# ZhongLingXiao/nano-kazen

Hardware: AMD Instinct MI355X
Metric: Msamples/s (w*h*spp/s) at 1920x1080, 1 M-tri scene (higher is better)
Workload: dtype f32

## Files before the change

nano-kazen_amd/csrc/kz_devfn.h:

```cpp
#pragma once
#include <hip/hip_runtime.h>
#include "kz_internal.h"
#include "kz_crmath.h"

#define KZ_BLOCK 256
#define KZ_INF __builtin_huge_valf()

struct V3 { float x, y, z; };
__device__ __forceinline__ V3 mk(float x, float y, float z) { V3 r; r.x = x; r.y = y; r.z = z; return r; }
__device__ __forceinline__ V3 mk(float a) { return mk(a, a, a); }
__device__ __forceinline__ V3 operator+(V3 a, V3 b) { return mk(a.x + b.x, a.y + b.y, a.z + b.z); }
__device__ __forceinline__ V3 operator-(V3 a, V3 b) { return mk(a.x - b.x, a.y - b.y, a.z - b.z); }
__device__ __forceinline__ V3 operator-(V3 a) { return mk(-a.x, -a.y, -a.z); }
__device__ __forceinline__ V3 operator*(V3 a, float s) { return mk(a.x * s, a.y * s, a.z * s); }
__device__ __forceinline__ V3 operator*(float s, V3 a) { return mk(a.x * s, a.y * s, a.z * s); }
__device__ __forceinline__ V3 operator*(V3 a, V3 b) { return mk(a.x * b.x, a.y * b.y, a.z * b.z); }
__device__ __forceinline__ V3 operator/(V3 a, float s) { return mk(a.x / s, a.y / s, a.z / s); }
__device__ __forceinline__ float dot(V3 a, V3 b) { return a.x * b.x + a.y * b.y + a.z * b.z; }
__device__ __forceinline__ V3 cross(V3 a, V3 b) { return mk(a.y * b.z - a.z * b.y, a.z * b.x - a.x * b.z, a.x * b.y - a.y * b.x); }
__device__ __forceinline__ float norm(V3 a) { return sqrtf(dot(a, a)); }
__device__ __forceinline__ V3 normalized(V3 a) { float n2 = dot(a, a); return n2 > 0.f ? a / sqrtf(n2) : a; }
__device__ __forceinline__ float maxCoeff(V3 a) { return fmaxf(a.x, fmaxf(a.y, a.z)); }
__device__ __forceinline__ float sqr(float x) { return x * x; }

// ... 64 lines not shown
    do {
        i ^= p; i *= 0xe170893d; i ^= p >> 16; i ^= (i & w) >> 4; i ^= p >> 8;
        i *= 0x0929eb3f; i ^= p >> 23; i ^= (i & w) >> 1; i *= 1 | p >> 27;
        i *= 0x6935fa69; i ^= (i & w) >> 11; i *= 0x74dcb303; i ^= (i & w) >> 2;
        i *= 0x9e501cc3; i ^= (i & w) >> 2; i *= 0xc860a3df; i &= w; i ^= i >> 5;
    } while (i >= l);
    if ((l & w) == 0) return (i + p) & w;
    return (i + p) % l;
}

struct Sampler {
    uint64_t state, inc;
    int px, py; uint32_t idx, dim;
    int type;
    uint64_t hp;

    __device__ __forceinline__ uint32_t nextUInt() {
        uint64_t old = state;
        state = old * PCG32_MULT + inc;
        uint32_t xs = (uint32_t)(((old >> 18u) ^ old) >> 27u);
        uint32_t rot = (uint32_t)(old >> 59u);
        return (xs >> rot) | (xs << ((~rot + 1u) & 31));
    }
    __device__ __forceinline__ float nextFloat() { return __uint_as_float((nextUInt() >> 9) | 0x3f800000u) - 1.0f; }
    __device__ __forceinline__ void generateSample(const KzParams &P, const KzDevTables &T, int x, int y, uint32_t sampleIndex) {
        px = x; py = y; idx = sampleIndex;
        hp = type != KZ_SAMPLER_INDEPENDENT ? hashPixelBlock(x, y) : 0ull;
        if (type != KZ_SAMPLER_PMJ02BN) {
            dim = 0;
            uint64_t h = hashPixelSeed(x, y, P.seed);
// ... 3 lines not shown
            state = state * PCG32_MULT + inc;
            KzPcgJump j = T.jump[sampleIndex];
            state = j.mult * state + inc * j.plus;
        } else {
            dim = 2;
        }
    }
    __device__ __forceinline__ float blueNoise(const KzDevTables &T, uint32_t tex) const {
        uint32_t t = tex % KZ_BLUENOISE_TEXTURES;
        uint32_t x = (uint32_t)px % KZ_BLUENOISE_RES, y = (uint32_t)py % KZ_BLUENOISE_RES;
        return T.bn[(t * KZ_BLUENOISE_RES + x) * KZ_BLUENOISE_RES + y];
    }
    __device__ __forceinline__ float next1D(const KzParams &P, const KzDevTables &T) {
        if (type == KZ_SAMPLER_INDEPENDENT) return nextFloat();
        if (type == KZ_SAMPLER_STRATIFIED) {
            const uint64_t h = hashDimSeed(hp, dim, P.seed);
            const int stratum = (int)permuteIdx(idx, P.sampleCount, (uint32_t)h);
            ++dim;
            const float delta = nextFloat();
            return ((float)stratum + delta) / (float)P.sampleCount;
        }
        if (type == KZ_SAMPLER_CORRELATED) {
            const uint64_t h = hashDimSeed(hp, dim, P.seed);
            const int p = (int)permuteIdx(idx, P.sampleCount, (uint32_t)h * 0x45fbe943u);
            const float j = nextFloat();
            ++dim;
            return ((float)p + j) / (float)P.sampleCount;
        }
        uint64_t h = hashDimSeed(hp, dim, P.seed);
        int index = (int)permuteIdx(idx, P.sampleCount, (uint32_t)h);
        float delta = blueNoise(T, dim);
        ++dim;
        const float num = (float)index + delta;
        return fminf(P.sppPow2 ? num * P.invSpp : num / (float)P.sampleCount, KZ_ONE_MINUS_EPS);
    }
    __device__ __forceinline__ void next2D(const KzParams &P, const KzDevTables &T, float &x, float &y) {
        if (type == KZ_SAMPLER_INDEPENDENT) { y = nextFloat(); x = nextFloat(); return; }
        if (type == KZ_SAMPLER_STRATIFIED) {
            const uint64_t h = hashDimSeed(hp, dim, P.seed);
            const int stratum = (int)permuteIdx(idx, P.sampleCount, (uint32_t)h);
            dim += 2;
            const int sx = stratum % P.resX, sy = stratum / P.resX;
            const float dx = nextFloat();
            const float dy = nextFloat();
            x = ((float)sx + dx) / (float)P.resX; y = ((float)sy + dy) / (float)P.resX;
            return;
        }
        if (type == KZ_SAMPLER_CORRELATED) {
            const uint32_t h = (uint32_t)hashDimSeed(hp, dim, P.seed);
            const uint32_t s = permuteIdx(idx, P.sampleCount, h * 0x51633e2du);
            const uint32_t cy = s / (uint32_t)P.resX, cx = s % (uint32_t)P.resX;
            const uint32_t sx = permuteIdx(cx, (uint32_t)P.resX, h * 0x68bc21ebu);
            const uint32_t sy = permuteIdx(cy, (uint32_t)P.resY, h * 0x02e5be93u);
            const float jx = nextFloat();
            const float jy = nextFloat();
            dim += 2;
            x = ((float)cx + ((float)sy + jx) / (float)P.resY) / (float)P.resX;
            y = ((float)cy + ((float)sx + jy) / (float)P.resX) / (float)P.resY;
            return;
        }
        uint32_t index = idx;
        uint32_t inst = dim / 2;
        if (inst >= KZ_PMJ02BN_SETS) {
            uint64_t h = hashDimSeed(hp, dim, P.seed);
            index = permuteIdx(idx, P.sampleCount, (uint32_t)h);
        }
        inst %= KZ_PMJ02BN_SETS; index %= KZ_PMJ02BN_SAMPLES;
        const float2 e = reinterpret_cast<const float2 *>(T.pmj)[(size_t)inst * KZ_PMJ02BN_SAMPLES + index];
        float ux = e.x, uy = e.y;
        ux += blueNoise(T, dim); uy += blueNoise(T, dim + 1);
        if (ux >= 1) ux -= 1;
        if (uy >= 1) uy -= 1;
        dim += 2;
        x = fminf(ux, KZ_ONE_MINUS_EPS); y = fminf(uy, KZ_ONE_MINUS_EPS);
    }
    __device__ __forceinline__ void nextPixel2D(const KzParams &P, const KzDevTables &T, float &x, float &y) {
        if (type != KZ_SAMPLER_PMJ02BN) { next2D(P, T, x, y); return; }
        int tile = P.pixelTileSize;
        int tx = px % tile, ty = py % tile;
// ... 43 lines not shown
    const float4 *tp = reinterpret_cast<const float4 *>(tri);
    return triTestV(tp[0], tp[1], tp[2], o, d, tmin, tmax, t, u, v, gid);
}
typedef float kz_f4v __attribute__((ext_vector_type(4)));
__device__ __forceinline__ float4 kzLoadStream(const float4 *p) { const kz_f4v v = __builtin_nontemporal_load(reinterpret_cast<const kz_f4v *>(p)); return make_float4(v.x, v.y, v.z, v.w); }
__device__ __forceinline__ void kzStoreStream(float4 *p, float4 v) { const kz_f4v t = {v.x, v.y, v.z, v.w}; __builtin_nontemporal_store(t, reinterpret_cast<kz_f4v *>(p)); }
__device__ __forceinline__ uint32_t kzLoadStream(const uint32_t *p) { return __builtin_nontemporal_load(p); }

typedef __attribute__((address_space(3))) uint32_t KzLds32;
__device__ __forceinline__ uint32_t kzLdsAddr(const uint32_t *p) { return (uint32_t)(uintptr_t)(const KzLds32 *)p; }
__device__ __forceinline__ void kzLdsPut(uint32_t a, uint32_t v) { *(KzLds32 *)(uintptr_t)a = v; }
__device__ __forceinline__ uint32_t kzLdsGet(uint32_t a) { return *(const KzLds32 *)(uintptr_t)a; }

struct Node4Test { uint32_t k0, k1, k2, k3; uint4 refs; };
typedef float kz_f2 __attribute__((ext_vector_type(2)));
__device__ __forceinline__ void node4KeysOf(const uint4 q0, const uint4 q1, const uint4 q2, V3 o, float rx, float ry, float rz, float tmin, float tmax,
                                            uint32_t (&key)[4]) {
    const float ax = __uint_as_float(q0.w) * rx, ay = __uint_as_float(q2.z) * ry, az = __uint_as_float(q2.w) * rz;
    const float bx = (__uint_as_float(q0.x) - o.x) * rx, by = (__uint_as_float(q0.y) - o.y) * ry, bz = (__uint_as_float(q0.z) - o.z) * rz;
    const uint32_t nX = rx >= 0.f ? q1.x : q1.w, fX = rx >= 0.f ? q1.w : q1.x;
    const uint32_t nY = ry >= 0.f ? q1.y : q2.x, fY = ry >= 0.f ? q2.x : q1.y;
    const uint32_t nZ = rz >= 0.f ? q1.z : q2.y, fZ = rz >= 0.f ? q2.y : q1.z;
    const kz_f2 AX = {ax, ax}, AY = {ay, ay}, AZ = {az, az}, BX = {bx, bx}, BY = {by, by}, BZ = {bz, bz};
#pragma unroll
    for (int i = 0; i < 4; ++i) {
        const kz_f2 qx = {(float)((nX >> (8 * i)) & 0xffu), (float)((fX >> (8 * i)) & 0xffu)};
        const kz_f2 qy = {(float)((nY >> (8 * i)) & 0xffu), (float)((fY >> (8 * i)) & 0xffu)};
        const kz_f2 qz = {(float)((nZ >> (8 * i)) & 0xffu), (float)((fZ >> (8 * i)) & 0xffu)};
        const kz_f2 tx = __builtin_elementwise_fma(qx, AX, BX), ty = __builtin_elementwise_fma(qy, AY, BY), tz = __builtin_elementwise_fma(qz, AZ, BZ);
        const float n = fmaxf(fmaxf(fmaxf(tx.x, ty.x), tz.x), tmin);
        const float f = fminf(fminf(fminf(tx.y, ty.y), tz.y) * 1.0000004f, tmax);
        key[i] = (n <= f) ? ((__float_as_uint(n) & ~3u) | (uint32_t)i) : 0xFFFFFFFFu;
    }
}
__device__ __forceinline__ const uint4 *kzNode4Ptr(const KzDevTables &T, uint32_t node) {
    return reinterpret_cast<const uint4 *>(reinterpret_cast<const char *>(T.nodes4) + (uint32_t)(node << 6));
}
__device__ __forceinline__ void node4Keys(const KzDevTables &T, uint32_t node, V3 o, float rx, float ry, float rz, float tmin, float tmax,
                                          uint32_t (&key)[4], uint4 &refs) {
    const uint4 *np = kzNode4Ptr(T, node);
    const uint4 q0 = np[0], q1 = np[1], q2 = np[2];
    refs = np[3];
    node4KeysOf(q0, q1, q2, o, rx, ry, rz, tmin, tmax, key);
}
__device__ __forceinline__ Node4Test node4Test(const KzDevTables &T, uint32_t node, V3 o, float rx, float ry, float rz, float tmin, float tmax) {
    Node4Test r; uint32_t key[4];
    node4Keys(T, node, o, rx, ry, rz, tmin, tmax, key, r.refs);
    uint32_t a = min(key[0], key[1]), b = max(key[0], key[1]), c = min(key[2], key[3]), d = max(key[2], key[3]);
    uint32_t lo = min(a, c), m1 = max(a, c), m2 = min(b, d), hi = max(b, d);
    r.k0 = lo; r.k1 = min(m1, m2); r.k2 = max(m1, m2); r.k3 = hi;
    return r;
}
__device__ __forceinline__ uint32_t pick4b(const uint4 &v, uint32_t i) {
    const bool b0 = i & 1u, b1 = i & 2u;
    const uint32_t lo = b0 ? v.y : v.x, hi = b0 ? v.w : v.z;
    return b1 ? hi : lo;
}
__device__ __forceinline__ uint32_t pick4(const uint4 &v, uint32_t i) { return i == 0 ? v.x : (i == 1 ? v.y : (i == 2 ? v.z : v.w)); }

__device__ __forceinline__ bool rayIsFinite(V3 o, V3 d) { return fabsf(o.x) + fabsf(o.y) + fabsf(o.z) + fabsf(d.x) + fabsf(d.y) + fabsf(d.z) < KZ_INF; }

template <bool STATS>
__device__ __forceinline__ bool closestHit(const KzDevTables &T, uint32_t rootRef, V3 o, V3 d, float tmin, float tmax,
                                           RawHit &best, uint32_t *stk, Counters &cn) {
    bool found = false;
    best.t = KZ_INF; best.u = best.v = 0.f; best.tri = 0; best.gid = 0;
    if (STATS) cn.rays++;
    if (rootRef == 0xFFFFFFFFu) return false;
    if (!(fabsf(o.x) + fabsf(o.y) + fabsf(o.z) + fabsf(d.x) + fabsf(d.y) + fabsf(d.z) < KZ_INF)) return false;
    const float rx = rcpExact(d.x), ry = rcpExact(d.y), rz = rcpExact(d.z);
    uint32_t cur = rootRef;
// ... 971 lines not shown
```

nano-kazen_amd/csrc/kz_render.hip:

```cpp
#include <hip/hip_runtime.h>

#include "kz_internal.h"
#include "kz_devfn.h"
#include "kz_wavefront.h"
#include "kz_integrators.h"
#include "kz_plan.h"
#include <algorithm>
#include <atomic>
#include <chrono>
#include <cmath>
#include <cstdio>
#include <cstdlib>
#include <cstring>
#include <mutex>
#include <string>
#include <thread>
#include <vector>

template <bool STATS, int EXT>
__global__ __launch_bounds__(KZ_BLOCK) void kz_path_megakernel(KzParams P, KzDevTables T, const uint32_t *__restrict__ pixList,
                                                               uint32_t nItems, uint32_t S, uint32_t sampleBegin, const uint32_t *__restrict__ itemSample,
                                                               float *__restrict__ outJx, float *__restrict__ outJy, float *__restrict__ outR,
                                                               float *__restrict__ outG, float *__restrict__ outB,
                                                               unsigned long long *__restrict__ stats) {
// ... 560 lines not shown
                HIP_TRY(hipStreamSynchronize(stream));
                if (left == 0) break;
            }
            trace(0, nextQ, nextCount, 0u, nextCount + 2, nullptr, nullptr);
            { int rc_ = stageMark(c, stream, 1); if (rc_) return rc_; }
            cur = nextQ; curCount = nextCount;
        }
    } else {
        const bool beside = P.nLights > 0 && maxDepth > 1 && (shadowBeside == 2 || (shadowBeside == 0 && items <= KZ_BESIDE_ITEMS));
        ds->lastInfo.shadowBeside = beside ? 1u : 0u;
        if (beside && !c.side) {
            HIP_TRY(hipStreamCreateWithFlags(&c.side, hipStreamNonBlocking));
            HIP_TRY(hipEventCreateWithFlags(&c.evFork, hipEventDisableTiming));
            HIP_TRY(hipEventCreateWithFlags(&c.evJoin, hipEventDisableTiming));
        }
        for (int iter = 0; iter < maxDepth; ++iter) {
            uint32_t *nextQ = W.queue[iter & 1], *nextCount = W.counts + 4 * (iter + 1), *shQ = W.queue[2], *shCount = W.counts + 4 * (iter + 1) + 1;
#define KZ_SHADE(ST, EX) hipLaunchKernelGGL((kz_wf_shade<ST, EX>), gShade, blk, 0, stream, P, Tsh, W, pixList, Sp, sBegin, iter, cur, curCount, items, nextQ, nextCount, shQ, shCount)
            const int xsel = P.bsdfExt == 0 ? 0 : (P.bsdfExt == KZ_X_MODELS ? KZ_X_MODELS : KZ_X_ALL);
            if (st) { if (xsel == KZ_X_ALL) KZ_SHADE(true, KZ_X_ALL); else if (xsel) KZ_SHADE(true, KZ_X_MODELS); else KZ_SHADE(true, 0); }
            else { if (xsel == KZ_X_ALL) KZ_SHADE(false, KZ_X_ALL); else if (xsel) KZ_SHADE(false, KZ_X_MODELS); else KZ_SHADE(false, 0); }
#undef KZ_SHADE
            const bool needExtend = iter < maxDepth - 1 || P.bgPresent;
            { int rc_ = stageMark(c, stream, 2); if (rc_) return rc_; }
            hipStream_t shOn = nullptr;
            if (beside && needExtend) {
                HIP_TRY(hipEventRecord(c.evFork, stream));
                HIP_TRY(hipStreamWaitEvent(c.side, c.evFork, 0));
                shOn = c.side;
            }
            if (P.nLights > 0) {
                if (P.shadowFast) {
                    uint32_t *litQ = W.queue[(iter & 1) ^ 1], *litCount = W.counts + 4 * 520 + 2 * (iter + 1), *litHead = litCount + 1;
// ... 470 lines not shown
```

nano-kazen_amd/csrc/kz_wavefront.h:

```cpp
#pragma once
#include "kz_state.h"
#include "kz_devfn.h"

#ifndef KZ_WF_QCAP
#define KZ_WF_QCAP 960
#endif
#define KZ_WF_ROUNDS (KZ_WF_QCAP / KZ_BLOCK)

struct WfAppender {
    uint32_t *s_buf; uint32_t *s_n; uint32_t *s_gb; uint32_t *gQueue; uint32_t *gCount;
    __device__ __forceinline__ void push(bool pred, uint32_t val) {
        const unsigned long long m = __ballot(pred);
        const int lane = threadIdx.x & 63;
        uint32_t base = 0;
        if (lane == 0 && m) base = atomicAdd(s_n, (uint32_t)__popcll(m));
        base = __shfl(base, 0, 64);
        if (pred) s_buf[base + __popcll(m & ((1ull << lane) - 1ull))] = val;
    }
    __device__ __forceinline__ void maybeFlush(bool force) {
        __syncthreads();
        const uint32_t n = *s_n;
        if (force ? (n > 0) : (n > KZ_WF_QCAP - KZ_BLOCK)) {
            if (threadIdx.x == 0) *s_gb = atomicAdd(gCount, n);
            __syncthreads();
// ... 18 lines not shown
__device__ __forceinline__ uint32_t wfPmjDim(const KzParams &P, int iter) {
    return 4u + (uint32_t)iter * (4u + (P.nLights > 0 ? 3u : 0u)) + (iter > 3 ? (uint32_t)(iter - 3) : 0u);
}
__device__ __forceinline__ void wfLoadSampler(const KzParams &P, const KzWf &W, uint32_t slot, int px, int py, uint32_t sampleIndex, Sampler &s, uint32_t dimPmj) {
    s.type = P.samplerType; s.px = px; s.py = py; s.idx = sampleIndex;
    if (P.samplerType == KZ_SAMPLER_PMJ02BN) {
        s.state = 0ull; s.inc = 0ull; s.dim = dimPmj; s.hp = hashPixelBlock(px, py);
        return;
    }
    const uint4 v = W.smp[slot];
    s.state = (uint64_t)v.x | ((uint64_t)v.y << 32);
    s.dim = (uint32_t)__builtin_amdgcn_readfirstlane((int)v.z);
    s.inc = (P.samplerType == KZ_SAMPLER_PMJ02BN) ? 0ull : ((hashPixelSeed(px, py, P.seed) << 1u) | 1u);
    s.hp = (P.samplerType != KZ_SAMPLER_INDEPENDENT) ? hashPixelBlock(px, py) : 0ull;
}
__device__ __forceinline__ void wfStoreSampler(const KzParams &P, const KzWf &W, uint32_t slot, const Sampler &s) {
    uint4 v;
    if (P.samplerType == KZ_SAMPLER_PMJ02BN) return;
    v.x = (uint32_t)s.state; v.y = (uint32_t)(s.state >> 32); v.z = s.dim; v.w = 0;
    W.smp[slot] = v;
}

__global__ __launch_bounds__(KZ_BLOCK) void kz_wf_generate(KzParams P, KzDevTables T, KzWf W, const uint32_t *__restrict__ pixList,
                                                           uint32_t nItems, uint32_t S, uint32_t sampleBegin) {
    const uint32_t item = blockIdx.x * KZ_BLOCK + threadIdx.x;
    if (item >= nItems) return;
    uint32_t pl, pxy;
    if ((S & 63u) == 0) { pl = (uint32_t)__builtin_amdgcn_readfirstlane((int)item) / S; pxy = (uint32_t)__builtin_amdgcn_readfirstlane((int)pixList[pl]); }
    else { pl = item / S; pxy = pixList[pl]; }
    const uint32_t so = item - pl * S;
// ... 87 lines not shown
            const int src = __ffsll(r) - 1;
            const V3 so = mk(__int_as_float(__builtin_amdgcn_readlane(__float_as_int(o.x), src)), __int_as_float(__builtin_amdgcn_readlane(__float_as_int(o.y), src)),
                             __int_as_float(__builtin_amdgcn_readlane(__float_as_int(o.z), src)));
            const V3 sd = mk(__int_as_float(__builtin_amdgcn_readlane(__float_as_int(d.x), src)), __int_as_float(__builtin_amdgcn_readlane(__float_as_int(d.y), src)),
                             __int_as_float(__builtin_amdgcn_readlane(__float_as_int(d.z), src)));
            const bool h = lane < n && triTestV(a, b, c, so, sd, tmin, KZ_INF, t, u, v, g);
            if (__ballot(h) != 0ull && lane == (uint32_t)src) hit = true;
        }
    } else if (cand) {
        for (uint32_t i = 0; i < n && !hit; ++i) hit = triTest(T.emTris + i, o, d, tmin, KZ_INF, t, u, v, g);
    }
    return hit;
}

template <bool STATS, int EXT>
__device__ __forceinline__ bool wfClassify(const KzParams &P, const KzDevTables &T, const KzWf &W, const uint32_t *__restrict__ pixList, uint32_t S, uint32_t sampleBegin,
                                           int iter, bool compact, uint32_t slot, Its &its, uint32_t &modelKey, Counters &cn, KzSst &sst) {
    bool survivor = false;
    const float4 h = kzLoadStream(&W.hit[slot]);
    const float4 rb = kzLoadStream(&W.rayB[slot]);
    const V3 rd = mk(rb.x, rb.y, rb.z);
#ifdef KZ_SHADESTAT
    sst.markw(10);
    if (h.x < KZ_INF) { const float4 *sp_ = reinterpret_cast<const float4 *>(T.shade + __float_as_uint(h.w)); const float4 a_ = sp_[0], b_ = sp_[6]; asm volatile("" :: "v"(a_.x), "v"(b_.x)); }
    sst.markw(11);
#endif
    if (!(h.x < KZ_INF)) {
        if (iter > 0 && P.bgPresent) {
            const float4 th = kzLoadStream(&W.thr[slot]);
            const V3 c = mk(th.x, th.y, th.z) * backgroundRadiance(P, T, rd);
            unsafeAtomicAdd(W.outR + slot, c.x); unsafeAtomicAdd(W.outG + slot, c.y); unsafeAtomicAdd(W.outB + slot, c.z);
        }
// ... 15 lines not shown
            const V3 c = (bsdfWeight * mk(th.x, th.y, th.z)) * mk(lr.radiance[0], lr.radiance[1], lr.radiance[2]);
            unsafeAtomicAdd(W.outR + slot, c.x); unsafeAtomicAdd(W.outG + slot, c.y); unsafeAtomicAdd(W.outB + slot, c.z);
        }
        return false;
    }
    const float wz = dot(-rd, its.sh.n);
    bool twoSided = false;
    if (EXT) {
        const int bt = T.bsdfs[its.bsdf].type;
        twoSided = bt == KZ_BSDF_DIELECTRIC || bt == KZ_BSDF_ROUGHDIELECTRIC || bt == KZ_BSDF_NORMALMAP;
        modelKey = (uint32_t)bt;
        if ((EXT & KZ_X_NMAP) && bt == KZ_BSDF_NORMALMAP) modelKey = 8u + ((uint32_t)T.bsdfs[T.bsdfs[its.bsdf].nested].type & 7u);
    }
    survivor = (wz > 0.f) || twoSided || isnan(wz);
    if (survivor && iter >= 3) {
        const uint32_t pl = slot / S; const uint32_t pxy = pixList[pl];
        Sampler smp; wfLoadSampler(P, W, slot, (int)(pxy & 0xffffu), (int)(pxy >> 16), sampleBegin + (slot - pl * S), smp, wfPmjDim(P, iter));
        const float4 th = kzLoadStream(&W.thr[slot]);
        V3 throughput = mk(th.x, th.y, th.z);
        const float etaA = compact ? 1.f : th.w;
        float probability;
        if (wfRouletteEnds(throughput, etaA, smp.next1D(P, T), probability)) survivor = false;
        else {
            throughput = throughput / probability;
            kzStoreStream(&W.thr[slot], make_float4(throughput.x, throughput.y, throughput.z, th.w));
            wfStoreSampler(P, W, slot, smp);
        }
    } else if (STATS && !survivor && P.nLights > 0) {
        bool alive = true;
        if (iter >= 3) {
            const uint32_t pl = slot / S; const uint32_t pxy = pixList[pl];
            Sampler smp; wfLoadSampler(P, W, slot, (int)(pxy & 0xffffu), (int)(pxy >> 16), sampleBegin + (slot - pl * S), smp, wfPmjDim(P, iter));
            const float4 th = kzLoadStream(&W.thr[slot]);
            const float etaA = compact ? 1.f : th.w;
            float probability;
            if (wfRouletteEnds(mk(th.x, th.y, th.z), etaA, smp.next1D(P, T), probability)) alive = false;
        }
        if (alive) cn.lsamples++;
    }
    return survivor;
}

template <bool STATS, int EXT>
__device__ __forceinline__ void wfShadeSurvivor(const KzParams &P, const KzDevTables &T, const KzWf &W, const uint32_t *__restrict__ pixList, uint32_t S, uint32_t sampleBegin,
                                                int iter, bool compact, uint32_t slot, const Its &its, bool &pushNext, bool &pushShadow, Counters &cn, KzSst &sst) {
    const float eps = P.traceBias;
    const float4 rb = kzLoadStream(&W.rayB[slot]);
    const V3 rd = mk(rb.x, rb.y, rb.z);
    float4 th = iter == 0 ? make_float4(1.f, 1.f, 1.f, 1.f) : kzLoadStream(&W.thr[slot]);
    V3 throughput = mk(th.x, th.y, th.z);
    const float eta = compact ? 1.f : th.w;
    float accRough = (iter == 0 || compact) ? 0.f : W.misc[slot].y;
    const uint32_t pl = slot / S;
    const uint32_t pxy = pixList[pl];
    Sampler smp; wfLoadSampler(P, W, slot, (int)(pxy & 0xffffu), (int)(pxy >> 16), sampleBegin + (slot - pl * S), smp, wfPmjDim(P, iter) + (iter >= 3 ? 1u : 0u));
    KzBSDF bsdf = T.bsdfs[its.bsdf];
    NMap nm; surfaceSetup<EXT>(T, its, bsdf, nm);
    const V3 wiLocal = toLocal(its.sh, -rd);
    sst.mark(2);
    const float pick = smp.next1D(P, T);
    if (P.nLights > 0) {
        const uint32_t li = min((uint32_t)floorf((float)P.nLights * pick), P.nLights - 1);
        const KzLightRow lrow = T.lights[li];
        if (STATS) cn.lsamples++;
        const LightSample ls = lightSample(T, lrow, its.p, [&]() { return smp.next1D(P, T); });
        const V3 lwi = ls.wi; const float dist = ls.dist, lpdf = ls.pdf;
        V3 Ls = ls.Ls;
        Ls = lightPickDivide(P, Ls);
        sst.mark(3);
        const V3 woL = toLocal(its.sh, lwi);
// ... 65 lines not shown
    __device__ __forceinline__ void flushAll() {
        const uint32_t nN = *s_nN, nS = *s_nS;
        if (threadIdx.x == 0) { if (nN) *s_gbN = atomicAdd(nextCount, nN); if (nS) *s_gbS = atomicAdd(shadowCount, nS); }
        __syncthreads();
        { const uint32_t gb = *s_gbN; for (uint32_t i = threadIdx.x; i < nN; i += KZ_BLOCK) nextQueue[gb + i] = s_bufN[i]; }
        { const uint32_t gb = *s_gbS; for (uint32_t i = threadIdx.x; i < nS; i += KZ_BLOCK) shadowQueue[gb + i] = s_bufS[i]; }
        __syncthreads();
        if (threadIdx.x == 0) { *s_nN = 0; *s_nS = 0; }
        __syncthreads();
    }
};

#define KZ_SV_CAP (2 * KZ_BLOCK)
template <bool STATS, int EXT>
__global__ __launch_bounds__(KZ_BLOCK, ((EXT & (KZ_X_TEX | KZ_X_NMAP)) ? 3 : KZ_SHADE_WAVES)) void kz_wf_shade(KzParams P, KzDevTables T, KzWf W, const uint32_t *__restrict__ pixList, uint32_t S,
                                                        uint32_t sampleBegin, int iter, const uint32_t *__restrict__ queue,
                                                        const uint32_t *__restrict__ countPtr, uint32_t countImm,
                                                        uint32_t *__restrict__ nextQueue, uint32_t *__restrict__ nextCount,
                                                        uint32_t *__restrict__ shadowQueue, uint32_t *__restrict__ shadowCount) {
    constexpr bool NMAPX = (EXT & KZ_X_NMAP) != 0;
    constexpr int SVW = NMAPX ? 19 : 16;
    constexpr uint32_t QCAP = (uint32_t)KZ_WF_QCAP;
    __shared__ uint32_t s_bufN[QCAP], s_bufS[QCAP]; __shared__ uint32_t s_nN, s_nS, s_gbN, s_gbS;
    constexpr bool SORT = NMAPX;
    __shared__ uint32_t s_hist[SORT ? 16 : 1]; __shared__ uint16_t s_perm[SORT ? KZ_BLOCK : 1];
    __shared__ uint32_t s_sv[SVW * KZ_SV_CAP]; __shared__ uint32_t s_svCnt[2];
    if (threadIdx.x == 0) { s_nN = 0; s_nS = 0; s_svCnt[0] = 0; s_svCnt[1] = 0; }
    if (SORT && threadIdx.x < 16) s_hist[threadIdx.x] = 0;
    __syncthreads();
    WfAppender apN = {s_bufN, &s_nN, &s_gbN, nextQueue, nextCount}, apS = {s_bufS, &s_nS, &s_gbS, shadowQueue, shadowCount};
    WfQueuePair qp = {s_bufN, s_bufS, &s_nN, &s_nS, &s_gbN, &s_gbS, nextQueue, nextCount, shadowQueue, shadowCount, QCAP};
// ... 1 lines not shown
    const int lane = threadIdx.x & 63;
    const bool compact = !EXT && !P.regularization;
    Counters cn = {0, 0, 0, 0, 0, 0};
    KzSst sst;
    uint32_t round = 0;
    for (uint32_t base = blockIdx.x * KZ_BLOCK;; base += gridDim.x * KZ_BLOCK, ++round) {
        const bool more = base < count;
        sst.mark(9);
        bool survivor = false;
        uint32_t slot = 0;
        Its its;
        uint32_t modelKey = 0;
        if (more && base + threadIdx.x < count) {
            const uint32_t qi = base + threadIdx.x;
            slot = queue ? queue[qi] : qi;
            survivor = wfClassify<STATS, EXT>(P, T, W, pixList, S, sampleBegin, iter, compact, slot, its, modelKey, cn, sst);
        }
        sst.mark(0);
        {
            const unsigned long long m = __ballot(survivor);
            uint32_t b = 0;
            if (lane == 0 && m) b = atomicAdd(&s_svCnt[round & 1u], (uint32_t)__popcll(m));
            b = __shfl(b, 0, 64);
            if (survivor) {
                const uint32_t e = b + __builtin_amdgcn_mbcnt_hi((uint32_t)(m >> 32), __builtin_amdgcn_mbcnt_lo((uint32_t)m, 0u));
                uint32_t *r = s_sv + e;
                r[0] = slot; r[KZ_SV_CAP] = __float_as_uint(its.p.x); r[2 * KZ_SV_CAP] = __float_as_uint(its.p.y); r[3 * KZ_SV_CAP] = __float_as_uint(its.p.z);
                r[4 * KZ_SV_CAP] = __float_as_uint(its.sh.s.x); r[5 * KZ_SV_CAP] = __float_as_uint(its.sh.s.y); r[6 * KZ_SV_CAP] = __float_as_uint(its.sh.s.z);
                r[7 * KZ_SV_CAP] = __float_as_uint(its.sh.t.x); r[8 * KZ_SV_CAP] = __float_as_uint(its.sh.t.y); r[9 * KZ_SV_CAP] = __float_as_uint(its.sh.t.z);
                r[10 * KZ_SV_CAP] = __float_as_uint(its.sh.n.x); r[11 * KZ_SV_CAP] = __float_as_uint(its.sh.n.y); r[12 * KZ_SV_CAP] = __float_as_uint(its.sh.n.z);
                r[13 * KZ_SV_CAP] = __float_as_uint(its.uvx); r[14 * KZ_SV_CAP] = __float_as_uint(its.uvy); r[15 * KZ_SV_CAP] = EXT ? (its.bsdf | (modelKey << 24)) : its.bsdf;
// ... 16 lines not shown
                for (uint32_t k = 0; k < (key & 15u); ++k) basePos += s_hist[k];
                s_perm[basePos + rank] = (uint16_t)threadIdx.x;
            }
            __syncthreads();
            if (threadIdx.x < take) mine = s_perm[threadIdx.x];
        }
        if (threadIdx.x < take) {
            const uint32_t *r = s_sv + (n0 - take) + mine;
            slot = r[0];
            its.p = mk(__uint_as_float(r[KZ_SV_CAP]), __uint_as_float(r[2 * KZ_SV_CAP]), __uint_as_float(r[3 * KZ_SV_CAP]));
            its.sh.s = mk(__uint_as_float(r[4 * KZ_SV_CAP]), __uint_as_float(r[5 * KZ_SV_CAP]), __uint_as_float(r[6 * KZ_SV_CAP]));
            its.sh.t = mk(__uint_as_float(r[7 * KZ_SV_CAP]), __uint_as_float(r[8 * KZ_SV_CAP]), __uint_as_float(r[9 * KZ_SV_CAP]));
            its.sh.n = mk(__uint_as_float(r[10 * KZ_SV_CAP]), __uint_as_float(r[11 * KZ_SV_CAP]), __uint_as_float(r[12 * KZ_SV_CAP]));
            its.uvx = __uint_as_float(r[13 * KZ_SV_CAP]); its.uvy = __uint_as_float(r[14 * KZ_SV_CAP]); its.bsdf = EXT ? (r[15 * KZ_SV_CAP] & 0xFFFFFFu) : r[15 * KZ_SV_CAP];
            if (NMAPX) its.dpdu = mk(__uint_as_float(r[16 * KZ_SV_CAP]), __uint_as_float(r[17 * KZ_SV_CAP]), __uint_as_float(r[18 * KZ_SV_CAP]));
            wfShadeSurvivor<STATS, EXT>(P, T, W, pixList, S, sampleBegin, iter, compact, slot, its, pushNext, pushShadow, cn, sst);
        }
        sst.mark(7);
        apN.push(pushNext, slot); apS.push(pushShadow, slot);
        __syncthreads();
        if (SORT && threadIdx.x < 16) s_hist[threadIdx.x] = 0;
        qp.flush(false);
        sst.mark(8);
        if (!more && n0 - take == 0) break;
        if (!more) base -= gridDim.x * KZ_BLOCK;
    }
    __syncthreads();
    qp.flush(true);
    if (STATS) wfStatsFlush(W.stats, cn, 0);
    sst.flush(W.stats);
}
// ... 4 lines not shown
#define KZ_TRACE_WAVES 8
#endif
template <int MODE, bool STATS>
__global__ __launch_bounds__(KZ_BLOCK) __attribute__((amdgpu_waves_per_eu(STATS ? KZ_TRACE_WAVES - 1 : KZ_TRACE_WAVES, STATS ? KZ_TRACE_WAVES - 1 : KZ_TRACE_WAVES)))
void kz_wf_trace(KzParams P, KzDevTables T, KzWf W, const uint32_t *__restrict__ queue,
                                                        const uint32_t *__restrict__ countPtr, uint32_t countImm, uint32_t *__restrict__ head, KzTune tune,
                                                        uint32_t *__restrict__ queueB, uint32_t *__restrict__ countPtrB) {
    extern __shared__ uint32_t s_stack[];
    const uint32_t count = countPtr ? *countPtr : countImm;
    [[maybe_unused]] constexpr bool SHADOW = MODE == 2 || MODE == 4;
    constexpr int kind = MODE == 4 ? 2 : MODE;
    const int lane = threadIdx.x & 63;
    constexpr uint32_t rowB = KZ_BLOCK * 4u;
    const uint32_t stkBase = kzLdsAddr(s_stack + threadIdx.x), ldsRows = (uint32_t)tune.ldsStack * rowB;
    uint32_t top = stkBase;
    uint32_t *const ovfBase = tune.ovf;
    const uint32_t ovfLane = blockIdx.x * KZ_BLOCK + threadIdx.x;
    const size_t ovfStride = tune.ovfStride;
#define ovf(row) ovfBase[(size_t)(row) * ovfStride + ovfLane]
    auto push = [&](uint32_t v) {
        const uint32_t dB = top - stkBase;
        if (dB < ldsRows) kzLdsPut(top, v); else ovf((dB - ldsRows) / rowB) = v;
        top += rowB;
    };
    const uint32_t root = P.rootRef4;
    const float eps = P.traceBias;
    Counters cn = {0, 0, 0, 0, 0, 0};
    const uint32_t nWaves = gridDim.x * (KZ_BLOCK / 64), waveId = blockIdx.x * (KZ_BLOCK / 64) + (threadIdx.x >> 6);
    const uint32_t batch = max(64u, min((uint32_t)tune.batch, ((count + nWaves - 1) / nWaves + 63u) & ~63u));
    const bool staticOnly = (unsigned long long)nWaves * batch >= count;
// ... 105 lines not shown
                poolNext += take;
            }
        }
        KZ_TST(0);
        if (!__any(active)) { if (exhausted) break; continue; }
        for (;;) {
            const bool inner = active && !(cur & 0x80000000u);
            const unsigned long long im = __ballot(inner);
            if (im == 0) break;
            if (__popcll(im) < tune.postpone && __ballot(active && (cur & 0x80000000u)) != 0) break;
#ifdef KZ_LANESTAT
            lsNodeIters++; lsInnerAtNode += __popcll(im); lsActiveAtNode += __popcll(__ballot(active));
#endif
            if (inner) {
                if (STATS) cn.nodes++;
                uint32_t key[4]; uint4 refs;
                node4Keys(T, cur, o, rx, ry, rz, tmin, tmax, key, refs);
                const uint32_t kmin = min(min(key[0], key[1]), min(key[2], key[3]));
                const bool any = kmin != 0xFFFFFFFFu;
                const uint32_t nxt = pick4b(refs, kmin);
                const bool p0 = key[0] != 0xFFFFFFFFu && key[0] != kmin, p1 = key[1] != 0xFFFFFFFFu && key[1] != kmin;
                const bool p2 = key[2] != 0xFFFFFFFFu && key[2] != kmin, p3 = key[3] != 0xFFFFFFFFu && key[3] != kmin;
                if (top - stkBase + 3u * rowB <= ldsRows) {
                    uint32_t a = top;
                    kzLdsPut(a, refs.x); a += p0 ? rowB : 0u;
                    kzLdsPut(a, refs.y); a += p1 ? rowB : 0u;
                    kzLdsPut(a, refs.z); a += p2 ? rowB : 0u;
                    kzLdsPut(a, refs.w); a += p3 ? rowB : 0u;
                    top = a;
                } else {
                    if (p0) push(refs.x);
                    if (p1) push(refs.y);
                    if (p2) push(refs.z);
                    if (p3) push(refs.w);
                }
                if (any) cur = nxt;
                else if (!popNext()) finish();
            }
        }
        KZ_TST(1);
#ifdef KZ_LANESTAT
        { const unsigned long long lm = __ballot(active && (cur & 0x80000000u)); if (lm) { lsLeafPhases++; lsLeafLanes += __popcll(lm);
          uint32_t mc = (active && (cur & 0x80000000u)) ? (cur & 7u) + 1 : 0; for (int off = 32; off > 0; off >>= 1) mc = max(mc, (uint32_t)__shfl_xor((int)mc, off, 64)); lsTriIters += mc; } }
#endif
        if (active && (cur & 0x80000000u)) {
            const uint32_t start = (cur & 0x7fffffffu) >> 3, cnt = (cur & 7u) + 1;
            bool occluded = false;
            for (uint32_t i = 0; i < cnt; ++i) {
                float t, u, v; uint32_t g;
// ... 65 lines not shown
        const V3 o = mk(a.x, a.y, a.z), d = mk(b.x, b.y, b.z);
        const float tmin = a.w;
        const bool live = have && root != 0xFFFFFFFFu && rayIsFinite(o, d);
        float tmax = live ? b.w : -KZ_INF;
        const float rx = rcpExact(fabsf(d.x) < 1e-20f ? copysignf(1e-20f, d.x) : d.x);
        const float ry = rcpExact(fabsf(d.y) < 1e-20f ? copysignf(1e-20f, d.y) : d.y);
        const float rz = rcpExact(fabsf(d.z) < 1e-20f ? copysignf(1e-20f, d.z) : d.z);
        bool found = false; float bt = KZ_INF, bu = 0.f, bv = 0.f; uint32_t bgid = 0;
        if (STATS && have) cn.rays++;
        if (__ballot(live) != 0ull) {
            uint32_t cur = root;
            int sp = 0;
            uint32_t stk0 = 0, stk1 = 0;
            for (;;) {
                if (!(cur & 0x80000000u)) {
                    uint32_t key[4]; uint4 refs;
                    node4Keys(T, cur, o, rx, ry, rz, tmin, tmax, key, refs);
                    if (STATS && live) cn.nodes++;
                    const unsigned long long m0 = __ballot(key[0] != 0xFFFFFFFFu), m1 = __ballot(key[1] != 0xFFFFFFFFu),
                                             m2 = __ballot(key[2] != 0xFFFFFFFFu), m3 = __ballot(key[3] != 0xFFFFFFFFu);
                    const unsigned long long any = m0 | m1 | m2 | m3;
                    bool descended = false;
                    if (any != 0ull) {
                        const int rep = __ffsll((long long)any) - 1;
                        uint32_t k0 = (uint32_t)__builtin_amdgcn_readlane((int)key[0], rep), k1 = (uint32_t)__builtin_amdgcn_readlane((int)key[1], rep),
                                 k2 = (uint32_t)__builtin_amdgcn_readlane((int)key[2], rep), k3 = (uint32_t)__builtin_amdgcn_readlane((int)key[3], rep);
                        k0 = m0 ? min(k0, 0xFFFFFFF8u) : 0xFFFFFFFFu; k1 = m1 ? min(k1, 0xFFFFFFF9u) : 0xFFFFFFFFu;
                        k2 = m2 ? min(k2, 0xFFFFFFFAu) : 0xFFFFFFFFu; k3 = m3 ? min(k3, 0xFFFFFFFBu) : 0xFFFFFFFFu;
                        const uint32_t r0 = (uint32_t)__builtin_amdgcn_readfirstlane((int)refs.x), r1 = (uint32_t)__builtin_amdgcn_readfirstlane((int)refs.y),
                                       r2 = (uint32_t)__builtin_amdgcn_readfirstlane((int)refs.z), r3 = (uint32_t)__builtin_amdgcn_readfirstlane((int)refs.w);
                        uint32_t ka = k0, kb = k1, kc = k2, kd = k3, ra = r0, rb = r1, rc = r2, rd = r3;
#define KZ_CSWAP(x, y, rx_, ry_) do { const bool s_ = y < x; const uint32_t tx_ = s_ ? y : x, ty_ = s_ ? x : y, tr_ = s_ ? ry_ : rx_, ts_ = s_ ? rx_ : ry_; x = tx_; y = ty_; rx_ = tr_; ry_ = ts_; } while (0)
                        KZ_CSWAP(ka, kb, ra, rb); KZ_CSWAP(kc, kd, rc, rd); KZ_CSWAP(ka, kc, ra, rc); KZ_CSWAP(kb, kd, rb, rd); KZ_CSWAP(kb, kc, rb, rc);
#undef KZ_CSWAP
                        auto pushEntry = [&](uint32_t ks, uint32_t ref) {
// ... 252 lines not shown
```

Measured before the change: 1929.

## Micro-optimize BVH traversal selects, shade divisions, and wave-uniform sampler hashing

Several independent micro-optimizations. Slot-to-pixel division becomes a host-precomputed multiply-shift. Sampler pixel hashing is computed once per wave when all lanes share a pixel. BVH node tests return explicit hit flags used for ballots and push predicates instead of comparing keys against a sentinel. The traversal loop also uses a raw v_min, a mask-based child pick, and a precomputed LDS stack-room bound. Together these aim to shave ALU work from the traversal and shading inner loops, while adding register pressure and inline-asm constraints that may hinder the compiler.

```diff
diff --git a/nano-kazen_amd/csrc/kz_devfn.h b/nano-kazen_amd/csrc/kz_devfn.h
--- a/nano-kazen_amd/csrc/kz_devfn.h
+++ b/nano-kazen_amd/csrc/kz_devfn.h
@@ -102,6 +102,12 @@
     int px, py; uint32_t idx, dim;
     int type;
     uint64_t hp;
+    bool uni = false;
+    uint64_t hpS = 0ull;
+    __device__ __forceinline__ uint64_t dimHash(const KzParams &P) const {
+        if (uni) return hashDimSeed(hpS, dim, P.seed);
+        return hashDimSeed(hp, dim, P.seed);
+    }
 
     __device__ __forceinline__ uint32_t nextUInt() {
         uint64_t old = state;
@@ -135,20 +141,20 @@
     __device__ __forceinline__ float next1D(const KzParams &P, const KzDevTables &T) {
         if (type == KZ_SAMPLER_INDEPENDENT) return nextFloat();
         if (type == KZ_SAMPLER_STRATIFIED) {
-            const uint64_t h = hashDimSeed(hp, dim, P.seed);
+            const uint64_t h = dimHash(P);
             const int stratum = (int)permuteIdx(idx, P.sampleCount, (uint32_t)h);
             ++dim;
             const float delta = nextFloat();
             return ((float)stratum + delta) / (float)P.sampleCount;
         }
         if (type == KZ_SAMPLER_CORRELATED) {
-            const uint64_t h = hashDimSeed(hp, dim, P.seed);
+            const uint64_t h = dimHash(P);
             const int p = (int)permuteIdx(idx, P.sampleCount, (uint32_t)h * 0x45fbe943u);
             const float j = nextFloat();
             ++dim;
             return ((float)p + j) / (float)P.sampleCount;
         }
-        uint64_t h = hashDimSeed(hp, dim, P.seed);
+        uint64_t h = dimHash(P);
         int index = (int)permuteIdx(idx, P.sampleCount, (uint32_t)h);
         float delta = blueNoise(T, dim);
         ++dim;
@@ -158,7 +164,7 @@
     __device__ __forceinline__ void next2D(const KzParams &P, const KzDevTables &T, float &x, float &y) {
         if (type == KZ_SAMPLER_INDEPENDENT) { y = nextFloat(); x = nextFloat(); return; }
         if (type == KZ_SAMPLER_STRATIFIED) {
-            const uint64_t h = hashDimSeed(hp, dim, P.seed);
+            const uint64_t h = dimHash(P);
             const int stratum = (int)permuteIdx(idx, P.sampleCount, (uint32_t)h);
             dim += 2;
             const int sx = stratum % P.resX, sy = stratum / P.resX;
@@ -168,7 +174,7 @@
             return;
         }
         if (type == KZ_SAMPLER_CORRELATED) {
-            const uint32_t h = (uint32_t)hashDimSeed(hp, dim, P.seed);
+            const uint32_t h = (uint32_t)dimHash(P);
             const uint32_t s = permuteIdx(idx, P.sampleCount, h * 0x51633e2du);
             const uint32_t cy = s / (uint32_t)P.resX, cx = s % (uint32_t)P.resX;
             const uint32_t sx = permuteIdx(cx, (uint32_t)P.resX, h * 0x68bc21ebu);
@@ -183,7 +189,7 @@
         uint32_t index = idx;
         uint32_t inst = dim / 2;
         if (inst >= KZ_PMJ02BN_SETS) {
-            uint64_t h = hashDimSeed(hp, dim, P.seed);
+            uint64_t h = dimHash(P);
             index = permuteIdx(idx, P.sampleCount, (uint32_t)h);
         }
         inst %= KZ_PMJ02BN_SETS; index %= KZ_PMJ02BN_SAMPLES;
@@ -257,8 +263,9 @@
 
 struct Node4Test { uint32_t k0, k1, k2, k3; uint4 refs; };
 typedef float kz_f2 __attribute__((ext_vector_type(2)));
+__device__ __forceinline__ float kzMinRaw(float a, float b) { float r; asm("v_min_f32 %0, %1, %2" : "=v"(r) : "v"(a), "v"(b)); return r; }
 __device__ __forceinline__ void node4KeysOf(const uint4 q0, const uint4 q1, const uint4 q2, V3 o, float rx, float ry, float rz, float tmin, float tmax,
-                                            uint32_t (&key)[4]) {
+                                            uint32_t (&key)[4], bool (&hit)[4]) {
     const float ax = __uint_as_float(q0.w) * rx, ay = __uint_as_float(q2.z) * ry, az = __uint_as_float(q2.w) * rz;
     const float bx = (__uint_as_float(q0.x) - o.x) * rx, by = (__uint_as_float(q0.y) - o.y) * ry, bz = (__uint_as_float(q0.z) - o.z) * rz;
     const uint32_t nX = rx >= 0.f ? q1.x : q1.w, fX = rx >= 0.f ? q1.w : q1.x;
@@ -272,19 +279,30 @@
         const kz_f2 qz = {(float)((nZ >> (8 * i)) & 0xffu), (float)((fZ >> (8 * i)) & 0xffu)};
         const kz_f2 tx = __builtin_elementwise_fma(qx, AX, BX), ty = __builtin_elementwise_fma(qy, AY, BY), tz = __builtin_elementwise_fma(qz, AZ, BZ);
         const float n = fmaxf(fmaxf(fmaxf(tx.x, ty.x), tz.x), tmin);
-        const float f = fminf(fminf(fminf(tx.y, ty.y), tz.y) * 1.0000004f, tmax);
-        key[i] = (n <= f) ? ((__float_as_uint(n) & ~3u) | (uint32_t)i) : 0xFFFFFFFFu;
-    }
+        const float f = kzMinRaw(fminf(fminf(tx.y, ty.y), tz.y) * 1.0000004f, tmax);
+        hit[i] = n <= f;
+        key[i] = hit[i] ? ((__float_as_uint(n) & ~3u) | (uint32_t)i) : 0xFFFFFFFFu;
+    }
+}
+__device__ __forceinline__ void node4KeysOf(const uint4 q0, const uint4 q1, const uint4 q2, V3 o, float rx, float ry, float rz, float tmin, float tmax,
+                                            uint32_t (&key)[4]) {
+    bool hit[4];
+    node4KeysOf(q0, q1, q2, o, rx, ry, rz, tmin, tmax, key, hit);
 }
 __device__ __forceinline__ const uint4 *kzNode4Ptr(const KzDevTables &T, uint32_t node) {
     return reinterpret_cast<const uint4 *>(reinterpret_cast<const char *>(T.nodes4) + (uint32_t)(node << 6));
 }
 __device__ __forceinline__ void node4Keys(const KzDevTables &T, uint32_t node, V3 o, float rx, float ry, float rz, float tmin, float tmax,
-                                          uint32_t (&key)[4], uint4 &refs) {
+                                          uint32_t (&key)[4], bool (&hit)[4], uint4 &refs) {
     const uint4 *np = kzNode4Ptr(T, node);
     const uint4 q0 = np[0], q1 = np[1], q2 = np[2];
     refs = np[3];
-    node4KeysOf(q0, q1, q2, o, rx, ry, rz, tmin, tmax, key);
+    node4KeysOf(q0, q1, q2, o, rx, ry, rz, tmin, tmax, key, hit);
+}
+__device__ __forceinline__ void node4Keys(const KzDevTables &T, uint32_t node, V3 o, float rx, float ry, float rz, float tmin, float tmax,
+                                          uint32_t (&key)[4], uint4 &refs) {
+    bool hit[4];
+    node4Keys(T, node, o, rx, ry, rz, tmin, tmax, key, hit, refs);
 }
 __device__ __forceinline__ Node4Test node4Test(const KzDevTables &T, uint32_t node, V3 o, float rx, float ry, float rz, float tmin, float tmax) {
     Node4Test r; uint32_t key[4];
@@ -298,6 +316,10 @@
     const bool b0 = i & 1u, b1 = i & 2u;
     const uint32_t lo = b0 ? v.y : v.x, hi = b0 ? v.w : v.z;
     return b1 ? hi : lo;
+}
+__device__ __forceinline__ uint32_t pick4m(uint32_t v0, uint32_t v1, uint32_t v2, uint32_t v3, bool ne0, bool ne1, bool ne2) {
+    const uint32_t a = ne2 ? v3 : v2, b = ne1 ? a : v1;
+    return ne0 ? b : v0;
 }
 __device__ __forceinline__ uint32_t pick4(const uint4 &v, uint32_t i) { return i == 0 ? v.x : (i == 1 ? v.y : (i == 2 ? v.z : v.w)); }
 
diff --git a/nano-kazen_amd/csrc/kz_render.hip b/nano-kazen_amd/csrc/kz_render.hip
--- a/nano-kazen_amd/csrc/kz_render.hip
+++ b/nano-kazen_amd/csrc/kz_render.hip
@@ -598,9 +598,13 @@
             HIP_TRY(hipEventCreateWithFlags(&c.evFork, hipEventDisableTiming));
             HIP_TRY(hipEventCreateWithFlags(&c.evJoin, hipEventDisableTiming));
         }
+        if (items > 0x80000000u || Sp == 0) return kz_fail(KZ_ERR_INVALID_ARG, "a pass of %u items x %u samples per pixel", items, Sp);
+        uint32_t sMul = 0, sShift = 0;
+        while ((2u << sShift) <= Sp && sShift < 31) ++sShift;
+        if (Sp & (Sp - 1)) sMul = (uint32_t)((((uint64_t)1 << (32 + sShift)) / Sp) + 1);
         for (int iter = 0; iter < maxDepth; ++iter) {
             uint32_t *nextQ = W.queue[iter & 1], *nextCount = W.counts + 4 * (iter + 1), *shQ = W.queue[2], *shCount = W.counts + 4 * (iter + 1) + 1;
-#define KZ_SHADE(ST, EX) hipLaunchKernelGGL((kz_wf_shade<ST, EX>), gShade, blk, 0, stream, P, Tsh, W, pixList, Sp, sBegin, iter, cur, curCount, items, nextQ, nextCount, shQ, shCount)
+#define KZ_SHADE(ST, EX) hipLaunchKernelGGL((kz_wf_shade<ST, EX>), gShade, blk, 0, stream, P, Tsh, W, pixList, Sp, sMul, sShift, sBegin, iter, cur, curCount, items, nextQ, nextCount, shQ, shCount)
             const int xsel = P.bsdfExt == 0 ? 0 : (P.bsdfExt == KZ_X_MODELS ? KZ_X_MODELS : KZ_X_ALL);
             if (st) { if (xsel == KZ_X_ALL) KZ_SHADE(true, KZ_X_ALL); else if (xsel) KZ_SHADE(true, KZ_X_MODELS); else KZ_SHADE(true, 0); }
             else { if (xsel == KZ_X_ALL) KZ_SHADE(false, KZ_X_ALL); else if (xsel) KZ_SHADE(false, KZ_X_MODELS); else KZ_SHADE(false, 0); }
diff --git a/nano-kazen_amd/csrc/kz_wavefront.h b/nano-kazen_amd/csrc/kz_wavefront.h
--- a/nano-kazen_amd/csrc/kz_wavefront.h
+++ b/nano-kazen_amd/csrc/kz_wavefront.h
@@ -56,6 +56,24 @@
     s.inc = (P.samplerType == KZ_SAMPLER_PMJ02BN) ? 0ull : ((hashPixelSeed(px, py, P.seed) << 1u) | 1u);
     s.hp = (P.samplerType != KZ_SAMPLER_INDEPENDENT) ? hashPixelBlock(px, py) : 0ull;
 }
+template <bool WAVE>
+__device__ __forceinline__ void wfLoadSamplerWave(const KzParams &P, const KzWf &W, uint32_t slot, uint32_t pxy, uint32_t sampleIndex, Sampler &s, uint32_t dimPmj) {
+    const int px = (int)(pxy & 0xffffu), py = (int)(pxy >> 16);
+    if (!WAVE || P.samplerType == KZ_SAMPLER_INDEPENDENT) { wfLoadSampler(P, W, slot, px, py, sampleIndex, s, dimPmj); return; }
+    const uint32_t first = (uint32_t)__builtin_amdgcn_readfirstlane((int)pxy);
+    const bool uni = __ballot(pxy != first) == 0ull;
+    s.type = P.samplerType; s.px = px; s.py = py; s.idx = sampleIndex;
+    s.uni = uni;
+    s.hpS = hashPixelBlock((int)(first & 0xffffu), (int)(first >> 16));
+    s.hp = 0ull;
+    if (!uni) s.hp = hashPixelBlock(px, py);
+    if (P.samplerType == KZ_SAMPLER_PMJ02BN) { s.state = 0ull; s.inc = 0ull; s.dim = dimPmj; return; }
+    const uint4 v = W.smp[slot];
+    s.state = (uint64_t)v.x | ((uint64_t)v.y << 32);
+    s.dim = (uint32_t)__builtin_amdgcn_readfirstlane((int)v.z);
+    s.inc = (hashPixelSeed(px, py, P.seed) << 1u) | 1u;
+}
+__device__ __forceinline__ uint32_t wfDivS(uint32_t slot, uint32_t mul, uint32_t shift) { return (mul ? __umulhi(slot, mul) : slot) >> shift; }
 __device__ __forceinline__ void wfStoreSampler(const KzParams &P, const KzWf &W, uint32_t slot, const Sampler &s) {
     uint4 v;
     if (P.samplerType == KZ_SAMPLER_PMJ02BN) return;
@@ -173,8 +191,8 @@
 }
 
 template <bool STATS, int EXT>
-__device__ __forceinline__ bool wfClassify(const KzParams &P, const KzDevTables &T, const KzWf &W, const uint32_t *__restrict__ pixList, uint32_t S, uint32_t sampleBegin,
-                                           int iter, bool compact, uint32_t slot, Its &its, uint32_t &modelKey, Counters &cn, KzSst &sst) {
+__device__ __forceinline__ bool wfClassify(const KzParams &P, const KzDevTables &T, const KzWf &W, const uint32_t *__restrict__ pixList, uint32_t S, uint32_t sMul, uint32_t sShift,
+                                           uint32_t sampleBegin, int iter, bool compact, uint32_t slot, Its &its, uint32_t &modelKey, Counters &cn, KzSst &sst) {
     bool survivor = false;
     const float4 h = kzLoadStream(&W.hit[slot]);
     const float4 rb = kzLoadStream(&W.rayB[slot]);
@@ -220,8 +238,8 @@
     }
     survivor = (wz > 0.f) || twoSided || isnan(wz);
     if (survivor && iter >= 3) {
-        const uint32_t pl = slot / S; const uint32_t pxy = pixList[pl];
-        Sampler smp; wfLoadSampler(P, W, slot, (int)(pxy & 0xffffu), (int)(pxy >> 16), sampleBegin + (slot - pl * S), smp, wfPmjDim(P, iter));
+        const uint32_t pl = wfDivS(slot, sMul, sShift); const uint32_t pxy = pixList[pl];
+        Sampler smp; wfLoadSamplerWave<EXT == 0 && !STATS>(P, W, slot, pxy, sampleBegin + (slot - pl * S), smp, wfPmjDim(P, iter));
         const float4 th = kzLoadStream(&W.thr[slot]);
         V3 throughput = mk(th.x, th.y, th.z);
         const float etaA = compact ? 1.f : th.w;
@@ -235,8 +253,8 @@
     } else if (STATS && !survivor && P.nLights > 0) {
         bool alive = true;
         if (iter >= 3) {
-            const uint32_t pl = slot / S; const uint32_t pxy = pixList[pl];
-            Sampler smp; wfLoadSampler(P, W, slot, (int)(pxy & 0xffffu), (int)(pxy >> 16), sampleBegin + (slot - pl * S), smp, wfPmjDim(P, iter));
+            const uint32_t pl = wfDivS(slot, sMul, sShift); const uint32_t pxy = pixList[pl];
+            Sampler smp; wfLoadSamplerWave<false>(P, W, slot, pxy, sampleBegin + (slot - pl * S), smp, wfPmjDim(P, iter));
             const float4 th = kzLoadStream(&W.thr[slot]);
             const float etaA = compact ? 1.f : th.w;
             float probability;
@@ -248,8 +266,8 @@
 }
 
 template <bool STATS, int EXT>
-__device__ __forceinline__ void wfShadeSurvivor(const KzParams &P, const KzDevTables &T, const KzWf &W, const uint32_t *__restrict__ pixList, uint32_t S, uint32_t sampleBegin,
-                                                int iter, bool compact, uint32_t slot, const Its &its, bool &pushNext, bool &pushShadow, Counters &cn, KzSst &sst) {
+__device__ __forceinline__ void wfShadeSurvivor(const KzParams &P, const KzDevTables &T, const KzWf &W, const uint32_t *__restrict__ pixList, uint32_t S, uint32_t sMul, uint32_t sShift,
+                                                uint32_t sampleBegin, int iter, bool compact, uint32_t slot, const Its &its, bool &pushNext, bool &pushShadow, Counters &cn, KzSst &sst) {
     const float eps = P.traceBias;
     const float4 rb = kzLoadStream(&W.rayB[slot]);
     const V3 rd = mk(rb.x, rb.y, rb.z);
@@ -257,9 +275,9 @@
     V3 throughput = mk(th.x, th.y, th.z);
     const float eta = compact ? 1.f : th.w;
     float accRough = (iter == 0 || compact) ? 0.f : W.misc[slot].y;
-    const uint32_t pl = slot / S;
+    const uint32_t pl = wfDivS(slot, sMul, sShift);
     const uint32_t pxy = pixList[pl];
-    Sampler smp; wfLoadSampler(P, W, slot, (int)(pxy & 0xffffu), (int)(pxy >> 16), sampleBegin + (slot - pl * S), smp, wfPmjDim(P, iter) + (iter >= 3 ? 1u : 0u));
+    Sampler smp; wfLoadSamplerWave<EXT == 0 && !STATS>(P, W, slot, pxy, sampleBegin + (slot - pl * S), smp, wfPmjDim(P, iter) + (iter >= 3 ? 1u : 0u));
     KzBSDF bsdf = T.bsdfs[its.bsdf];
     NMap nm; surfaceSetup<EXT>(T, its, bsdf, nm);
     const V3 wiLocal = toLocal(its.sh, -rd);
@@ -355,7 +373,7 @@
 #define KZ_SV_CAP (2 * KZ_BLOCK)
 template <bool STATS, int EXT>
 __global__ __launch_bounds__(KZ_BLOCK, ((EXT & (KZ_X_TEX | KZ_X_NMAP)) ? 3 : KZ_SHADE_WAVES)) void kz_wf_shade(KzParams P, KzDevTables T, KzWf W, const uint32_t *__restrict__ pixList, uint32_t S,
-                                                        uint32_t sampleBegin, int iter, const uint32_t *__restrict__ queue,
+                                                        uint32_t sMul, uint32_t sShift, uint32_t sampleBegin, int iter, const uint32_t *__restrict__ queue,
                                                         const uint32_t *__restrict__ countPtr, uint32_t countImm,
                                                         uint32_t *__restrict__ nextQueue, uint32_t *__restrict__ nextCount,
                                                         uint32_t *__restrict__ shadowQueue, uint32_t *__restrict__ shadowCount) {
@@ -387,7 +405,7 @@
         if (more && base + threadIdx.x < count) {
             const uint32_t qi = base + threadIdx.x;
             slot = queue ? queue[qi] : qi;
-            survivor = wfClassify<STATS, EXT>(P, T, W, pixList, S, sampleBegin, iter, compact, slot, its, modelKey, cn, sst);
+            survivor = wfClassify<STATS, EXT>(P, T, W, pixList, S, sMul, sShift, sampleBegin, iter, compact, slot, its, modelKey, cn, sst);
         }
         sst.mark(0);
         {
@@ -434,7 +452,7 @@
             its.sh.n = mk(__uint_as_float(r[10 * KZ_SV_CAP]), __uint_as_float(r[11 * KZ_SV_CAP]), __uint_as_float(r[12 * KZ_SV_CAP]));
             its.uvx = __uint_as_float(r[13 * KZ_SV_CAP]); its.uvy = __uint_as_float(r[14 * KZ_SV_CAP]); its.bsdf = EXT ? (r[15 * KZ_SV_CAP] & 0xFFFFFFu) : r[15 * KZ_SV_CAP];
             if (NMAPX) its.dpdu = mk(__uint_as_float(r[16 * KZ_SV_CAP]), __uint_as_float(r[17 * KZ_SV_CAP]), __uint_as_float(r[18 * KZ_SV_CAP]));
-            wfShadeSurvivor<STATS, EXT>(P, T, W, pixList, S, sampleBegin, iter, compact, slot, its, pushNext, pushShadow, cn, sst);
+            wfShadeSurvivor<STATS, EXT>(P, T, W, pixList, S, sMul, sShift, sampleBegin, iter, compact, slot, its, pushNext, pushShadow, cn, sst);
         }
         sst.mark(7);
         apN.push(pushNext, slot); apS.push(pushShadow, slot);
@@ -469,6 +487,7 @@
     constexpr uint32_t rowB = KZ_BLOCK * 4u;
     const uint32_t stkBase = kzLdsAddr(s_stack + threadIdx.x), ldsRows = (uint32_t)tune.ldsStack * rowB;
     uint32_t top = stkBase;
+    int32_t topRoom3 = (int32_t)(stkBase + ldsRows) - (int32_t)(3u * rowB); asm volatile("" : "+v"(topRoom3));
     uint32_t *const ovfBase = tune.ovf;
     const uint32_t ovfLane = blockIdx.x * KZ_BLOCK + threadIdx.x;
     const size_t ovfStride = tune.ovfStride;
@@ -604,25 +623,27 @@
 #endif
             if (inner) {
                 if (STATS) cn.nodes++;
-                uint32_t key[4]; uint4 refs;
-                node4Keys(T, cur, o, rx, ry, rz, tmin, tmax, key, refs);
+                uint32_t key[4]; bool hit[4]; uint4 refs;
+                node4Keys(T, cur, o, rx, ry, rz, tmin, tmax, key, hit, refs);
                 const uint32_t kmin = min(min(key[0], key[1]), min(key[2], key[3]));
                 const bool any = kmin != 0xFFFFFFFFu;
-                const uint32_t nxt = pick4b(refs, kmin);
-                const bool p0 = key[0] != 0xFFFFFFFFu && key[0] != kmin, p1 = key[1] != 0xFFFFFFFFu && key[1] != kmin;
-                const bool p2 = key[2] != 0xFFFFFFFFu && key[2] != kmin, p3 = key[3] != 0xFFFFFFFFu && key[3] != kmin;
-                if (top - stkBase + 3u * rowB <= ldsRows) {
+                const bool ne0 = key[0] != kmin, ne1 = key[1] != kmin, ne2 = key[2] != kmin, ne3 = key[3] != kmin;
+                uint32_t c0 = refs.x, c1 = refs.y, c2 = refs.z, c3 = refs.w;
+                asm volatile("" : "+v"(c0), "+v"(c1), "+v"(c2), "+v"(c3));
+                const uint32_t nxt = pick4m(c0, c1, c2, c3, ne0, ne1, ne2);
+                const bool p0 = hit[0] && ne0, p1 = hit[1] && ne1, p2 = hit[2] && ne2, p3 = hit[3] && ne3;
+                if ((int32_t)top <= topRoom3) {
                     uint32_t a = top;
-                    kzLdsPut(a, refs.x); a += p0 ? rowB : 0u;
-                    kzLdsPut(a, refs.y); a += p1 ? rowB : 0u;
-                    kzLdsPut(a, refs.z); a += p2 ? rowB : 0u;
-                    kzLdsPut(a, refs.w); a += p3 ? rowB : 0u;
+                    kzLdsPut(a, c0); a += p0 ? rowB : 0u;
+                    kzLdsPut(a, c1); a += p1 ? rowB : 0u;
+                    kzLdsPut(a, c2); a += p2 ? rowB : 0u;
+                    kzLdsPut(a, c3); a += p3 ? rowB : 0u;
                     top = a;
                 } else {
-                    if (p0) push(refs.x);
-                    if (p1) push(refs.y);
-                    if (p2) push(refs.z);
-                    if (p3) push(refs.w);
+                    if (p0) push(c0);
+                    if (p1) push(c1);
+                    if (p2) push(c2);
+                    if (p3) push(c3);
                 }
                 if (any) cur = nxt;
                 else if (!popNext()) finish();
@@ -718,11 +739,10 @@
             uint32_t stk0 = 0, stk1 = 0;
             for (;;) {
                 if (!(cur & 0x80000000u)) {
-                    uint32_t key[4]; uint4 refs;
-                    node4Keys(T, cur, o, rx, ry, rz, tmin, tmax, key, refs);
+                    uint32_t key[4]; bool hit[4]; uint4 refs;
+                    node4Keys(T, cur, o, rx, ry, rz, tmin, tmax, key, hit, refs);
                     if (STATS && live) cn.nodes++;
-                    const unsigned long long m0 = __ballot(key[0] != 0xFFFFFFFFu), m1 = __ballot(key[1] != 0xFFFFFFFFu),
-                                             m2 = __ballot(key[2] != 0xFFFFFFFFu), m3 = __ballot(key[3] != 0xFFFFFFFFu);
+                    const unsigned long long m0 = __ballot(hit[0]), m1 = __ballot(hit[1]), m2 = __ballot(hit[2]), m3 = __ballot(hit[3]);
                     const unsigned long long any = m0 | m1 | m2 | m3;
                     bool descended = false;
                     if (any != 0ull) {
```

Result: no change. 1929, median of 3 (+0.0%).
